# Healthcare-Robotics/assistive-gym

Hardware: NVIDIA H100
Metric: env-steps/sec FeedingJaco-v1 @batch4096 (higher is better)
Workload: dtype f32

## Files before the change

### assistive_gym_b200/capi.py

```python
import ctypes as C
import os

_HERE = os.path.dirname(os.path.abspath(__file__))
LIB_PATH = os.path.join(_HERE, 'csrc', 'libagphys.so')

P_I32 = C.POINTER(C.c_int32)
P_F64 = C.POINTER(C.c_double)
P_F32 = C.POINTER(C.c_float)


class AgConfig(C.Structure):
    _fields_ = [('dt', C.c_double), ('num_substeps', C.c_int), ('num_solver_iters', C.c_int),
                ('erp', C.c_double), ('contact_erp', C.c_double), ('linear_slop', C.c_double),
                ('residual_threshold', C.c_double), ('contact_threshold', C.c_double),
                ('linear_damping', C.c_double), ('angular_damping', C.c_double),
                ('max_coord_velocity', C.c_double), ('hull_margin', C.c_double),
                ('cone_friction', C.c_int), ('gyroscopic', C.c_int), ('max_contacts', C.c_int),
                ('warmstart_contact', C.c_double), ('warmstart_joint', C.c_double)]


def default_config(**kw):
    c = AgConfig(dt=0.02, num_substeps=1, num_solver_iters=50, erp=0.2, contact_erp=0.08, linear_slop=1e-5,
                 residual_threshold=1e-7, contact_threshold=0.02, linear_damping=0.04, angular_damping=0.04,
                 max_coord_velocity=100.0, hull_margin=0.001, cone_friction=1, gyroscopic=1, max_contacts=128,
# ... 228 lines not shown
    lib.ag_scratch_init.argtypes = [vp, C.POINTER(AgScratchParams), vp, vp, vp]
    lib.ag_scratch_step_dev.argtypes = [vp, vp, vp, vp, vp, vp]
    lib.ag_scratch_step_host.argtypes = [vp, vp, vp, vp, vp, vp]
    lib.ag_drinking_init.argtypes = [vp, C.POINTER(AgDrinkingParams), vp]
    lib.ag_drinking_step_dev.argtypes = [vp, vp, vp, vp, vp, vp]
    lib.ag_drinking_step_host.argtypes = [vp, vp, vp, vp, vp, vp]
    lib.ag_drinking_get_state.argtypes = [vp, vp, vp, vp]
    lib.ag_coop_init.argtypes = [vp, C.POINTER(AgCoopParams), vp, vp]
    lib.ag_coop_step_dev.argtypes = [vp, vp, vp, vp, vp, vp, vp]
    lib.ag_coop_step_host.argtypes = [vp, vp, vp, vp, vp, vp, vp]
    lib.ag_coop_classify.argtypes = [vp, ci, vp, vp]
    lib.ag_render.argtypes = [vp, C.POINTER(AgCamera), ci, vp, vp, vp]
    lib.ag_ik_solve.argtypes = [vp, ci, vp, ci, vp, vp, ci, ci, C.c_float, C.c_uint64, vp, vp, vp]
    lib.ag_state_size.restype = C.c_size_t
    lib.ag_state_size.argtypes = [vp]
    lib.ag_state_get.argtypes = [vp, vp]
    lib.ag_state_set.argtypes = [vp, vp]
    lib.ag_kernel_launches.restype = C.c_uint64
    lib.ag_kernel_launches.argtypes = [vp]
    lib.ag_overflow_count.argtypes = [vp]
    lib.ag_get_solver_stats.argtypes = [vp, vp, vp]
    lib.ag_get_pgs_cycles.argtypes = [vp, vp]
    lib.ag_get_pgs_trips.argtypes = [vp, vp, vp]
    lib.ag_get_pgs_occupancy.argtypes = [vp, vp, vp]
    lib.ag_profile_enable.argtypes = [vp, ci]
    lib.ag_profile_get.argtypes = [vp, ci, vp, ci, vp, vp]
    if path is None:
        _lib = lib
    return lib


EXPORTED_SYMBOLS = [
    'ag_last_error', 'ag_default_config', 'ag_create', 'ag_destroy', 'ag_num_envs', 'ag_stream',
    'ag_set_base_pose', 'ag_set_base_velocity', 'ag_set_joint_state', 'ag_set_link_friction',
    'ag_set_body_active', 'ag_forward_kinematics', 'ag_set_motor_host', 'ag_set_motor_targets_dev', 'ag_set_motor_targets_host',
    'ag_step', 'ag_get_joint_states', 'ag_get_link_states', 'ag_get_contacts', 'ag_contact_force_sum',
    'ag_closest_points', 'ag_feeding_init', 'ag_feeding_reset_episode', 'ag_feeding_set_tremor', 'ag_set_hard_limits', 'ag_feeding_step_dev', 'ag_ik_solve', 'ag_bathing_init', 'ag_bathing_step_dev', 'ag_bathing_step_host',
    'ag_feeding_step_host', 'ag_feeding_step_host_begin', 'ag_feeding_step_host_end', 'ag_state_size', 'ag_state_get', 'ag_state_set', 'ag_kernel_launches',
    'ag_cloth_init', 'ag_cloth_set_state', 'ag_cloth_get_state', 'ag_cloth_set_anchor', 'ag_cloth_anchor_follow', 'ag_cloth_set_gravity',
    'ag_cloth_get_contacts', 'ag_cloth_device_state', 'ag_scratch_init', 'ag_scratch_step_dev', 'ag_scratch_step_host', 'ag_render', 'ag_set_body_gravity', 'ag_get_link_aabb', 'ag_dressing_init', 'ag_dressing_reset_episode', 'ag_dressing_set_tremor', 'ag_set_motor_force_scale', 'ag_dressing_step_dev', 'ag_dressing_step_host',
    'ag_overflow_count', 'ag_get_solver_stats', 'ag_get_pgs_cycles', 'ag_get_pgs_trips', 'ag_get_pgs_occupancy', 'ag_profile_enable', 'ag_profile_get',
    'ag_coop_init', 'ag_coop_step_dev', 'ag_coop_step_host', 'ag_coop_classify', 'ag_bathing_set_target_frames',
    'ag_drinking_init', 'ag_drinking_step_dev', 'ag_drinking_step_host', 'ag_drinking_get_state',
]
```

### assistive_gym_b200/csrc/ag_device.cuh

```cuda
#pragma once
#include <string.h>
#include "ag_math.cuh"
#include "ag_types.h"

AG_HD float ld1(const float* p, int item, int N, int e) { return p[(size_t)item * N + e]; }
AG_HD void st1(float* p, int item, int N, int e, float v) { p[(size_t)item * N + e] = v; }
AG_HD f3 ld3(const float* p, int item, int N, int e) {
  size_t b = (size_t)item * 3 * N + e;
  return f3(p[b], p[b + N], p[b + 2 * (size_t)N]);
}
AG_HD void st3(float* p, int item, int N, int e, f3 v) {
  size_t b = (size_t)item * 3 * N + e;
  p[b] = v.x; p[b + N] = v.y; p[b + 2 * (size_t)N] = v.z;
}
AG_HD q4 ld4(const float* p, int item, int N, int e) {
  size_t b = (size_t)item * 4 * N + e;
  return q4(p[b], p[b + N], p[b + 2 * (size_t)N], p[b + 3 * (size_t)N]);
}
AG_HD void st4(float* p, int item, int N, int e, q4 v) {
  size_t b = (size_t)item * 4 * N + e;
  p[b] = v.x; p[b + N] = v.y; p[b + 2 * (size_t)N] = v.z; p[b + 3 * (size_t)N] = v.w;
}
AG_HD f3 tv3(const float* p, int i) { return f3(AG_LDG(p + 3 * i), AG_LDG(p + 3 * i + 1), AG_LDG(p + 3 * i + 2)); }
AG_HD q4 tv4(const float* p, int i) { return q4(AG_LDG(p + 4 * i), AG_LDG(p + 4 * i + 1), AG_LDG(p + 4 * i + 2), AG_LDG(p + 4 * i + 3)); }
// ... 98 lines not shown
AG_HD vq4 ldq4(const float* p) {
#if defined(__CUDA_ARCH__)
  float4 v = __ldg((const float4*)p); vq4 r; r.x = v.x; r.y = v.y; r.z = v.z; r.w = v.w; return r;
#else
  return *(const vq4*)p;
#endif
}
AG_HD int support4(const float* vq, int g0, int n, f3 d) {
  int bi = 0; float best = -3.0e38f;
  const int ng = (n + 3) >> 2;
  const float* p = vq + (size_t)g0 * 12;
  for (int g = 0; g < ng; g++, p += 12) {
    vq4 X = ldq4(p), Y = ldq4(p + 4), Z = ldq4(p + 8);
    float d0 = d.x * X.x + d.y * Y.x + d.z * Z.x, d1 = d.x * X.y + d.y * Y.y + d.z * Z.y;
    float d2 = d.x * X.z + d.y * Y.z + d.z * Z.z, d3v = d.x * X.w + d.y * Y.w + d.z * Z.w;
    if (d0 > best) { best = d0; bi = 4 * g; }
    if (d1 > best) { best = d1; bi = 4 * g + 1; }
    if (d2 > best) { best = d2; bi = 4 * g + 2; }
    if (d3v > best) { best = d3v; bi = 4 * g + 3; }
  }
  return bi < n ? bi : 0;
}

AG_HDN inline bool gjk_cores(const float* verts, const float* vq, int va0, int ga0, int nA, int vb0, int gb0, int nB, const m3& R, f3 t,
                             f3& pa, f3& pb, f3& nrm, float& dist) {
  d3 W[4]; f3 PA[4], PB[4];
  int IA[4], IB[4];
  double lam[4] = {1.0, 0.0, 0.0, 0.0};
  int n = 0;
  d3 v = to_d3(mul(R, tv3(verts, va0)) + t) - to_d3(tv3(verts, vb0));
  if (dot(v, v) < 1e-20) v = d3(1.0, 0.0, 0.0);
  bool overlap = false;
  double lower_bound = 0.0;
  for (int it = 0; it < 32; it++) {
    f3 vf = to_f3(v);
    f3 da = mulT(R, -vf);
    int ia = support4(vq, ga0, nA, da), ib = support4(vq, gb0, nB, vf);
    f3 sa = mul(R, tv3(verts, va0 + ia)) + t;
    f3 sb = tv3(verts, vb0 + ib);
    d3 w = to_d3(sa) - to_d3(sb);
    double vv = dot(v, v);
    double vw = dot(v, w);
    if (n > 0 && vw > 0.0) lower_bound = fmax(lower_bound, vw / sqrt(vv));
    if (n > 0 && vv - vw <= 1e-10 * vv) break;
    bool dup = false;
    for (int i = 0; i < n; i++) if (IA[i] == ia && IB[i] == ib) dup = true;
    if (dup) break;
    W[n] = w; PA[n] = sa; PB[n] = sb; IA[n] = ia; IB[n] = ib; n++;
    if (n == 1) { lam[0] = 1.0; }
    else if (n == 2) {
      double u, s; seg_origin(W[0], W[1], u, s);
      if (s <= 0.0) { n = 1; lam[0] = 1.0; }
      else if (u <= 0.0) { W[0] = W[1]; PA[0] = PA[1]; PB[0] = PB[1]; IA[0] = IA[1]; IB[0] = IB[1]; n = 1; lam[0] = 1.0; }
      else { lam[0] = u; lam[1] = s; }
    } else if (n == 3) {
      double l3[3]; tri_origin(W[0], W[1], W[2], l3[0], l3[1], l3[2]);
      int m = 0;
      for (int i = 0; i < 3; i++) if (l3[i] > 0.0) { W[m] = W[i]; PA[m] = PA[i]; PB[m] = PB[i]; IA[m] = IA[i]; IB[m] = IB[i]; lam[m] = l3[i]; m++; }
      n = m;
    } else {
      double bestd = 1e300; int bf = -1; double bl[3] = {0.0, 0.0, 0.0};
      double bestd_all = 1e300; int bf_all = 0; double bla[3] = {1.0, 0.0, 0.0};
      bool any_out = false;
      for (int f = 0; f < 4; f++) {
        int i0 = (f == 3) ? 1 : 0, i1 = (f == 0) ? 1 : ((f == 1) ? 2 : 3), i2 = (f == 0) ? 2 : ((f == 1) ? 3 : ((f == 2) ? 1 : 2)), i3 = (f == 0) ? 3 : ((f == 1) ? 1 : ((f == 2) ? 2 : 0));
        d3 a = W[i0], b = W[i1], c = W[i2], d = W[i3];
        d3 nn = cross(b - a, c - a);
        double sp = -dot(a, nn), sd = dot(d - a, nn);
        double nl = sqrt(dot(nn, nn));
        double tol_d = 1e-9 * nl * sqrt(dot(d - a, d - a)), tol_p = 1e-9 * nl * sqrt(dot(a, a));
        bool inside = (sp * sd > 0.0) && (fabs(sd) > tol_d) && (fabs(sp) > tol_p);
        double u, s, r; tri_origin(a, b, c, u, s, r);
        d3 pt = a * u + b * s + c * r;
        double dd = dot(pt, pt);
        if (dd < bestd_all) { bestd_all = dd; bf_all = f; bla[0] = u; bla[1] = s; bla[2] = r; }
        if (inside) continue;
        any_out = true;
        if (dd < bestd) { bestd = dd; bf = f; bl[0] = u; bl[1] = s; bl[2] = r; }
      }
      if (!any_out) {
        if (lower_bound <= 1e-7) { overlap = true; break; }
        bf = bf_all; bl[0] = bla[0]; bl[1] = bla[1]; bl[2] = bla[2];
      }
      int f = bf;
      int id[3];
      id[0] = (f == 3) ? 1 : 0; id[1] = (f == 0) ? 1 : ((f == 1) ? 2 : 3); id[2] = (f == 0) ? 2 : ((f == 1) ? 3 : ((f == 2) ? 1 : 2));
      d3 tw[3]; f3 ta[3], tb[3]; int tia[3], tib[3];
      for (int i = 0; i < 3; i++) { tw[i] = W[id[i]]; ta[i] = PA[id[i]]; tb[i] = PB[id[i]]; tia[i] = IA[id[i]]; tib[i] = IB[id[i]]; }
      int m = 0;
      for (int i = 0; i < 3; i++) if (bl[i] > 0.0) { W[m] = tw[i]; PA[m] = ta[i]; PB[m] = tb[i]; IA[m] = tia[i]; IB[m] = tib[i]; lam[m] = bl[i]; m++; }
      n = m;
    }
    d3 nv(0.0, 0.0, 0.0);
    for (int i = 0; i < n; i++) nv = nv + W[i] * lam[i];
    v = nv;
    if (dot(v, v) <= 1e-16) { overlap = true; break; }
  }
  if (overlap) return true;
  d3 qa(0.0, 0.0, 0.0), qb(0.0, 0.0, 0.0);
  for (int i = 0; i < n; i++) { qa = qa + to_d3(PA[i]) * lam[i]; qb = qb + to_d3(PB[i]) * lam[i]; }
  d3 d = qa - qb;
  double dn = sqrt(dot(d, d));
  pa = to_f3(qa); pb = to_f3(qb);
  dist = (float)dn;
  nrm = dn > 0.0 ? to_f3(d * (1.0 / dn)) : f3(0.f, 0.f, 1.f);
  return false;
}

AG_HDN inline void pen_faces(const SimDev& S, int va0, int nA, int pa0, int npA, int vb0, int nB, int pb0, int npB,
                             const m3& R, f3 t, f3& pa, f3& pb, f3& nrm, float& dist) {
  float best = -1e30f; bool found = false;
  for (int k = 0; k < npA; k++) {
    f3 nl; float dl; ld_plane(S.planes, pa0 + k, nl, dl);
    f3 n = mul(R, nl); float d = dl + dot(n, t);
    int jb = 0; float mn = dot(n, tv3(S.verts, vb0));
    for (int j = 1; j < nB; j++) { float x = dot(n, tv3(S.verts, vb0 + j)); if (x < mn) { mn = x; jb = j; } }
    float sep = mn - d;
    if (sep > best) { best = sep; found = true; nrm = -n; pb = tv3(S.verts, vb0 + jb); pa = pb - n * sep; }
  }
  for (int k = 0; k < npB; k++) {
    f3 n; float d; ld_plane(S.planes, pb0 + k, n, d);
    f3 nl = mulT(R, n);
    int ja = 0; float mn = dot(nl, tv3(S.verts, va0));
    for (int j = 1; j < nA; j++) { float x = dot(nl, tv3(S.verts, va0 + j)); if (x < mn) { mn = x; ja = j; } }
    float sep = mn + dot(n, t) - d;
    if (sep > best) { best = sep; found = true; nrm = n; pa = mul(R, tv3(S.verts, va0 + ja)) + t; pb = pa - n * sep; }
  }
  if (!found) { nrm = f3(0.f, 0.f, 1.f); pa = mul(R, tv3(S.verts, va0)) + t; pb = tv3(S.verts, vb0); best = 0.f; }
  dist = fminf(best, 0.f);
}

struct CandSet { NpOut c[4]; int n; };
struct CandSel {
  NpOut prim; NpOut pool[12]; int np;
};

AG_HDN inline void face_cands(const SimDev& S, int vv0, int nV, float rV, bool v_is_a, int p0, int np, float rP,
                              const m3& R, f3 t, f3 n_to_v, float d_primary, float tol, float max_dist, CandSel& cs) {
  int kf = -1; float best = 0.98f; f3 nf; float df = 0.f;
  for (int k = 0; k < np; k++) {
    f3 n; float d; ld_plane(S.planes, p0 + k, n, d);
    if (!v_is_a) { f3 nw = mul(R, n); d = d + dot(nw, t); n = nw; }
    float al = dot(n, n_to_v);
    if (al > best) { best = al; kf = k; nf = n; df = d; }
  }
  if (kf < 0) return;
  for (int i = 0; i < nV; i++) {
    f3 v = tv3(S.verts, vv0 + i);
    if (v_is_a) v = mul(R, v) + t;
    float h = dot(nf, v) - df;
    float d = h - rV - rP;
    if (d > d_primary + tol || d > max_dist) continue;
    f3 proj = v - nf * h;
    bool inside = true;
    for (int k = 0; k < np; k++) {
      if (k == kf) continue;
      f3 n; float dd; ld_plane(S.planes, p0 + k, n, dd);
      if (!v_is_a) { f3 nw = mul(R, n); dd = dd + dot(nw, t); n = nw; }
      if (dot(n, proj) - dd > 1e-6f) { inside = false; break; }
    }
    if (!inside) continue;
    if (cs.np >= 12) {
      int wi = 0; for (int q = 1; q < 12; q++) if (cs.pool[q].d > cs.pool[wi].d) wi = q;
      if (d >= cs.pool[wi].d) continue;
      cs.np = 12;
      NpOut& o = cs.pool[wi];
      f3 on_v = v - nf * rV, on_f = proj + nf * rP;
      if (v_is_a) { o.pa = on_v; o.pb = on_f; o.n = nf; } else { o.pa = on_f; o.pb = on_v; o.n = -nf; }
      o.d = d;
      continue;
    }
    NpOut& o = cs.pool[cs.np++];
    f3 on_v = v - nf * rV, on_f = proj + nf * rP;
    if (v_is_a) { o.pa = on_v; o.pb = on_f; o.n = nf; } else { o.pa = on_f; o.pb = on_v; o.n = -nf; }
    o.d = d;
  }
}

AG_HDN inline int select_cands(const CandSel& cs, NpOut* out) {
  if (cs.np == 0) { out[0] = cs.prim; return 1; }
  bool used[12];
  int first = 0;
  for (int i = 0; i < 12; i++) used[i] = i >= cs.np;
  for (int i = 1; i < cs.np; i++) if (cs.pool[i].d < cs.pool[first].d) first = i;
  int nc = 0; out[nc++] = cs.pool[first]; used[first] = true;
  while (nc < 4) {
    int bi = -1; float bd = 1e-8f;
    for (int i = 0; i < cs.np; i++) {
      if (used[i]) continue;
      float md = 1e30f;
      for (int k = 0; k < nc; k++) { f3 d = cs.pool[i].pa - out[k].pa; md = fminf(md, dot(d, d)); }
      if (md > bd) { bd = md; bi = i; }
    }
    if (bi < 0) break;
    used[bi] = true; out[nc++] = cs.pool[bi];
  }
  return nc;
}

AG_HDN inline int narrow_pair(const SimDev& S, int e, int ca, int cb, float max_dist, bool manifold, NpOut* out) {
  const int N = S.N;
  int ta = AG_LDG(S.col_type + ca), tb = AG_LDG(S.col_type + cb);
  float ra = AG_LDG(S.col_radius + ca), rb = AG_LDG(S.col_radius + cb);
  int ka = AG_LDG(S.col_link + ca), kb = AG_LDG(S.col_link + cb);
  int va0 = AG_LDG(S.col_v0 + ca), nA = AG_LDG(S.col_nv + ca), vb0 = AG_LDG(S.col_v0 + cb), nB = AG_LDG(S.col_nv + cb);
  int pa0 = AG_LDG(S.col_p0 + ca), npA = AG_LDG(S.col_np + ca), pb0 = AG_LDG(S.col_p0 + cb), npB = AG_LDG(S.col_np + cb);
  f3 posA = ld3(S.lpos, ka, N, e), posB = ld3(S.lpos, kb, N, e);
  q4 qA = ld4(S.lquat, ka, N, e), qB = ld4(S.lquat, kb, N, e);
  CandSel cs; cs.np = 0;
  int nout;
  if (ta == 3 || tb == 3) {
    if (ta == tb) return 0;
    bool flip = (ta == 3);
    q4 qP = flip ? qA : qB, qV = flip ? qB : qA;
    f3 pP = flip ? posA : posB, pV = flip ? posB : posA;
    m3 R = mul(transpose(qmat(qP)), qmat(qV));
    f3 t = qrot_inv(qP, pV - pP);
    int vv0 = flip ? vb0 : va0, nV = flip ? nB : nA; float rv = flip ? rb : ra;
    f3 pn; float pd; ld_plane(S.planes, flip ? pa0 : pb0, pn, pd);
    int j = 0; float mn = 1e30f;
    for (int i = 0; i < nV; i++) { float x = dot(pn, mul(R, tv3(S.verts, vv0 + i)) + t); if (x < mn) { mn = x; j = i; } }
    float d = mn - pd - rv;
    if (d > max_dist) return 0;
    f3 vj = mul(R, tv3(S.verts, vv0 + j)) + t;
    cs.prim.pa = vj - pn * rv; cs.prim.pb = vj - pn * (mn - pd); cs.prim.n = pn; cs.prim.d = d;
    if (manifold && nV > 1) face_cands(S, vv0, nV, rv, true, flip ? pa0 : pb0, 1, 0.f, R, t, pn, d, max_dist * 0.5f, max_dist, cs);
    nout = select_cands(cs, out);
    m3 RP = qmat(qP);
    for (int i = 0; i < nout; i++) {
      f3 a = mul(RP, out[i].pa) + pP, b = mul(RP, out[i].pb) + pP, n = mul(RP, out[i].n);
      if (!flip) { out[i].pa = a; out[i].pb = b; out[i].n = n; }
      else { out[i].pa = b; out[i].pb = a; out[i].n = -n; }
    }
    return nout;
  }
  m3 RB = qmat(qB);
  m3 R = mul(transpose(RB), qmat(qA));
  f3 t = mulT(RB, posA - posB);
  f3 pa, pb, nrm; float dist = 0.f;
  bool ov = gjk_cores(S.verts, S.vertq, va0, AG_LDG(S.col_g0 + ca), nA, vb0, AG_LDG(S.col_g0 + cb), nB, R, t, pa, pb, nrm, dist);
  if (ov) pen_faces(S, va0, nA, pa0, npA, vb0, nB, pb0, npB, R, t, pa, pb, nrm, dist);
  float d = dist - ra - rb;
  if (d > max_dist) return 0;
  cs.prim.n = nrm; cs.prim.pa = pa - nrm * ra; cs.prim.pb = pb + nrm * rb; cs.prim.d = d;
  if (manifold) {
    if (npB > 0 && nA > 1) face_cands(S, va0, nA, ra, true, pb0, npB, rb, R, t, nrm, d, max_dist * 0.5f, max_dist, cs);
    if (npA > 0 && nB > 1) face_cands(S, vb0, nB, rb, false, pa0, npA, ra, R, t, -nrm, d, max_dist * 0.5f, max_dist, cs);
  }
  nout = select_cands(cs, out);
  for (int i = 0; i < nout; i++) {
    out[i].pa = mul(RB, out[i].pa) + posB; out[i].pb = mul(RB, out[i].pb) + posB; out[i].n = mul(RB, out[i].n);
  }
  return nout;
}

AG_HD int ag_atomic_inc(int* p) {
#if defined(__CUDA_ARCH__)
  return atomicAdd(p, 1);
#else
  int v = *p; *p = v + 1; return v;
#endif
}
AG_HD int ag_atomic_add(int* p, int k) {
#if defined(__CUDA_ARCH__)
  return atomicAdd(p, k);
#else
  int v = *p; *p = v + k; return v;
#endif
}

AG_HDN inline void pairs_body(int tid, const SimDev& S, const KP& kp) {
  const int N = S.N;
  int Npad = kp.i0;
// ... 12 lines not shown
    float tha = AG_LDG(S.col_thresh + ca);
    if (!aabb_ov(amin, amax, lbmin, lbmax, fac * fminf(tha, tlb))) continue;
    for (int cb = cb0; cb < cb0 + ncb; cb++) {
      float thr = fac * fminf(tha, AG_LDG(S.col_thresh + cb));
      if (!aabb_ov(amin, amax, ld3(S.cmin, cb, N, e), ld3(S.cmax, cb, N, e), thr)) continue;
      int slot = ag_atomic_inc(S.cand_count + e);
      int cost = AG_LDG(S.col_nv + ca) + AG_LDG(S.col_nv + cb); if (cost > 255) cost = 255;
      if (slot < S.maxcand) S.cand[(size_t)slot * N + e] = ((unsigned)(255 - cost) << 24) | ((unsigned)ca * (unsigned)S.nc + (unsigned)cb);
    }
  }
}

AG_HDN inline void csort_body(int tid, const SimDev& S, const KP&) {
  const int N = S.N;
  int e = tid % N, cs = tid / N;
  int n = S.cand_count[e]; if (n > S.maxcand) n = S.maxcand;
  if (cs >= n) return;
  unsigned w = S.cand[(size_t)cs * N + e];
  int rank = 0;
  for (int j = 0; j < n; j++) rank += (S.cand[(size_t)j * N + e] < w) ? 1 : 0;
  S.cand_s[(size_t)rank * N + e] = w;
}

AG_HDN inline void narrow_body(int tid, const SimDev& S, const KP&) {
  const int N = S.N;
  int e = tid % N, cs = tid / N;
  int ncand = S.cand_count[e]; if (ncand > S.maxcand) ncand = S.maxcand;
  if (cs >= ncand) return;
  unsigned pk = S.cand_s[(size_t)cs * N + e] & 0xffffffu;
  int ca = (int)(pk / (unsigned)S.nc), cb = (int)(pk % (unsigned)S.nc);
  float thr = S.contact_thr * fminf(AG_LDG(S.col_thresh + ca), AG_LDG(S.col_thresh + cb));
  NpOut out[4];
  int n = narrow_pair(S, e, ca, cb, thr, true, out);
  for (int i = 0; i < n; i++) {
    int slot = ag_atomic_inc(S.c_count + e);
    if (slot >= S.maxraw) continue;
    S.c_key[(size_t)slot * N + e] = pk * 4u + (unsigned)i;
    float* c = S.c_data + (size_t)slot * AG_CFR * N + e;
    c[(size_t)CF_PAX * N] = out[i].pa.x; c[(size_t)CF_PAY * N] = out[i].pa.y; c[(size_t)CF_PAZ * N] = out[i].pa.z;
    c[(size_t)CF_PBX * N] = out[i].pb.x; c[(size_t)CF_PBY * N] = out[i].pb.y; c[(size_t)CF_PBZ * N] = out[i].pb.z;
    c[(size_t)CF_NX * N] = out[i].n.x; c[(size_t)CF_NY * N] = out[i].n.y; c[(size_t)CF_NZ * N] = out[i].n.z;
    c[(size_t)CF_DIST * N] = out[i].d;
  }
}

AG_HD void contact_refs(const SimDev& S, int e, unsigned key, int& refA, int& refB);
AG_HDN inline void sort_body(int tid, const SimDev& S, const KP&) {
  const int N = S.N;
  int e = tid % N, slot = tid / N;
  int cnt = S.c_count[e];
  int n = cnt < S.maxraw ? cnt : S.maxraw;
  if (slot == 0 && ((cnt > S.maxc) || (S.cand_count[e] > S.maxcand))) S.overflow[e] = 1;
  if (slot >= n) return;
  unsigned key = S.c_key[(size_t)slot * N + e];
  int rank = 0;
  for (int j = 0; j < n; j++) rank += (S.c_key[(size_t)j * N + e] < key) ? 1 : 0;
  if (rank >= S.maxc) return;
  S.s_key[(size_t)rank * N + e] = key;
  { int ra, rb2; contact_refs(S, e, key, ra, rb2); S.s_ref[(size_t)rank * 4 * N + e] = ra; S.s_ref[((size_t)rank * 4 + 1) * N + e] = rb2; }
  for (int f = 0; f <= CF_DIST; f++) cf_st(S.s_data, rank, f, N, e, S.c_data[((size_t)slot * AG_CFR + f) * N + e]);
}

struct AI { s3 A; m3 B; s3 D; };
struct SVf { f3 a, l; };

AG_HD SVf ai_mul(const AI& I, SVf v) {
  SVf r;
// ... 226 lines not shown
```

### assistive_gym_b200/csrc/agphys.cu

```cuda
#include <stdio.h>
#include <stdlib.h>
#include <string.h>
#include <string>
#include <vector>
#include <algorithm>
#include "../../include/agphys.h"
#include "ag_device.cuh"
#include "ag_solver.cuh"
#include "ag_feeding.cuh"
#include "ag_bathing.cuh"
#include "ag_ik.cuh"
#include "ag_cloth.cuh"
#include "ag_dressing.cuh"
#include "ag_render.cuh"
#include "ag_scratch.cuh"
#include "ag_coop.cuh"
#include "ag_drinking.cuh"

#ifndef AG_CPU_EMU
#include <cuda_runtime.h>
#define AG_GLOBAL __global__
#else
#define AG_GLOBAL
typedef void* cudaStream_t;
// ... 8 lines not shown
    int tid = blockIdx.x * blockDim.x + threadIdx.x;                            \
    if (tid < p.n) body(tid, S, p);                                             \
  }
#else
#define AG_KERNEL(name, body) \
  static void name(SimDev S, KP p) { for (int tid = 0; tid < p.n; tid++) body(tid, S, p); }
#endif

#ifndef AG_CPU_EMU
#define AG_KERNEL_B(name, body, minblocks)                                      \
  __global__ void __launch_bounds__(128, minblocks) name(SimDev S, KP p) {      \
    int tid = blockIdx.x * blockDim.x + threadIdx.x;                            \
    if (tid < p.n) body(tid, S, p);                                             \
  }
#else
#define AG_KERNEL_B(name, body, minblocks) AG_KERNEL(name, body)
#endif
AG_KERNEL(k_fk, fk_body)
AG_KERNEL(k_aabb, aabb_body)
AG_KERNEL(k_linkaabb, linkaabb_body)
AG_KERNEL(k_pairs, pairs_body)
AG_KERNEL(k_csort, csort_body)
AG_KERNEL_B(k_narrow, narrow_body, 3)
AG_KERNEL(k_sort, sort_body)
AG_KERNEL(k_dyn, dyn_body)
AG_KERNEL(k_rows, rows_body)
AG_KERNEL(k_crows, crows_body)
#ifndef AG_CPU_EMU
__global__ void __launch_bounds__(32) k_pgs(SimDev S, KP p) {
  extern __shared__ __align__(128) float pgs_smem[];
  pgs_warp(S, pgs_smem, p.i0, blockIdx.x * RS_CTA_ENVS);
}
__global__ void __launch_bounds__(1024) k_order(SimDev S, KP) {
  __shared__ int hist[64];
  if (threadIdx.x < 64) hist[threadIdx.x] = 0;
  __syncthreads();
  for (int e = threadIdx.x; e < S.N; e += blockDim.x) atomicAdd(&hist[pgs_work_bucket(S, e)], 1);
  __syncthreads();
  if (threadIdx.x == 0) { int acc = 0; for (int b = 0; b < 64; b++) { int c = hist[b]; hist[b] = acc; acc += c; } }
  __syncthreads();
  for (int e = threadIdx.x; e < S.N; e += blockDim.x) S.pgs_order[atomicAdd(&hist[pgs_work_bucket(S, e)], 1)] = e;
}
#else
static void k_pgs(SimDev S, KP p) {
  std::vector<float> buf((size_t)rs_env_floats(S) + 8);
  float* base = (float*)(((uintptr_t)buf.data() + 15) & ~(uintptr_t)15);
// ... 883 lines not shown
    const float* o = in + sz * e;
    for (int b = 0; b < s->nb; b++) {
      for (int a = 0; a < 3; a++) { bp[((size_t)b * 3 + a) * N + e] = o[a]; bl[((size_t)b * 3 + a) * N + e] = o[7 + a]; ba[((size_t)b * 3 + a) * N + e] = o[10 + a]; }
      for (int a = 0; a < 4; a++) bq[((size_t)b * 4 + a) * N + e] = o[3 + a];
      o += 13;
    }
    for (int k = 0; k < s->nl; k++) { q[(size_t)k * N + e] = o[0]; qd[(size_t)k * N + e] = o[1]; o += 2; }
  }
  if (h2d(s, s->S.base_pos, bp.data(), bp.size() * 4) || h2d(s, s->S.base_quat, bq.data(), bq.size() * 4) ||
      h2d(s, s->S.base_lin, bl.data(), bl.size() * 4) || h2d(s, s->S.base_ang, ba.data(), ba.size() * 4) ||
      h2d(s, s->S.jq, q.data(), q.size() * 4) || h2d(s, s->S.jqd, qd.data(), qd.size() * 4)) return -1;
  run_fk_all(s);
  return 0;
}

int ag_get_pgs_cycles(AgSim* s, int32_t* cycles) {
  DevGuard guard__(s->device); return d2h(s, cycles, s->S.pgs_cycles, sizeof(int) * s->S.N); }
int ag_get_pgs_trips(AgSim* s, int32_t* trips, int32_t* stream_floats) {
  DevGuard guard__(s->device);
  if (trips && d2h(s, trips, s->S.pgs_trips, sizeof(int) * s->S.N)) return -1;
  if (stream_floats && d2h(s, stream_floats, s->S.rs_nfloats, sizeof(int) * s->S.N)) return -1;
  return 0;
}
int ag_get_pgs_occupancy(AgSim* s, int32_t* ctas_per_sm, int32_t* smem_bytes) {
  DevGuard guard__(s->device);
  const size_t smem = (size_t)rs_cta_floats(s->S) * sizeof(float);
  int ctas = 0;
#ifndef AG_CPU_EMU
  if (cudaOccupancyMaxActiveBlocksPerMultiprocessor(&ctas, k_pgs, 32, smem) != cudaSuccess) return fail("cudaOccupancyMaxActiveBlocksPerMultiprocessor(k_pgs) failed");
#endif
  if (ctas_per_sm) *ctas_per_sm = ctas;
  if (smem_bytes) *smem_bytes = (int32_t)smem;
  return 0;
}

int ag_get_solver_stats(AgSim* s, int32_t* contacts, int32_t* iters) {
  DevGuard guard__(s->device);
  if (contacts && d2h(s, contacts, s->S.c_count, sizeof(int) * s->S.N)) return -1;
  if (iters && d2h(s, iters, s->S.iters_used, sizeof(int) * s->S.N)) return -1;
  return 0;
}

int ag_overflow_count(AgSim* s) {
  DevGuard guard__(s->device);
  std::vector<int> o(s->S.N);
  if (d2h(s, o.data(), s->S.overflow, sizeof(int) * s->S.N)) return -1;
// ... 843 lines not shown
```

### assistive_gym_b200/sim.py

```python
import ctypes as C

import numpy as np

from . import capi


def _p(a):
    return None if a is None else a.ctypes.data_as(C.c_void_p)


def _f32(a, shape=None):
    if a is None:
        return None
    a = np.asarray(a, dtype=np.float32)
    if shape is not None:
        a = np.broadcast_to(a, shape)
    return np.ascontiguousarray(a)


def _i32(a):
    return None if a is None else np.ascontiguousarray(a, dtype=np.int32)


_OBS_W = {'feeding': (25, 23), 'scratch': (30, 34), 'bathing': (24, 28), 'dressing': (24, 28), 'drinking': (25, 0)}
# ... 130 lines not shown

    def kernel_launches(self):
        return int(self.lib.ag_kernel_launches(self.h))

    def overflow_count(self):
        return int(self.lib.ag_overflow_count(self.h))

    def solver_stats(self):
        c, it = np.zeros(self.n, dtype=np.int32), np.zeros(self.n, dtype=np.int32)
        self._ck(self.lib.ag_get_solver_stats(self.h, _p(c), _p(it)))
        return c, it

    def pgs_cycles(self):
        c = np.zeros(self.n, dtype=np.int32)
        self._ck(self.lib.ag_get_pgs_cycles(self.h, _p(c)))
        return c

    def pgs_trips(self):
        t = np.zeros(self.n, dtype=np.int32)
        f = np.zeros(self.n, dtype=np.int32)
        self._ck(self.lib.ag_get_pgs_trips(self.h, _p(t), _p(f)))
        return t, f

    def pgs_occupancy(self):
        c, b = C.c_int32(0), C.c_int32(0)
        self._ck(self.lib.ag_get_pgs_occupancy(self.h, C.byref(c), C.byref(b)))
        return c.value, b.value

    def profile_enable(self, on=True):
        self._ck(self.lib.ag_profile_enable(self.h, int(bool(on))))

    def profile_get(self):
        mx, stride = 32, 48
        names = C.create_string_buffer(mx * stride)
        ms = np.zeros(mx, dtype=np.float32)
        cnt = np.zeros(mx, dtype=np.int32)
        n = self.lib.ag_profile_get(self.h, mx, names, stride, _p(ms), _p(cnt))
        out = {}
        for i in range(max(n, 0)):
            nm = names.raw[i * stride:(i + 1) * stride].split(b'\0')[0].decode()
            out[nm] = (float(ms[i]), int(cnt[i]))
        return out

    def stream_ptr(self):
        return int(self.lib.ag_stream(self.h) or 0)

# ... 233 lines not shown
```

### include/agphys.h

```cpp
#ifndef AGPHYS_H
#define AGPHYS_H
#include <stddef.h>
#include <stdint.h>

#ifdef __cplusplus
extern "C" {
#endif

enum { AG_JOINT_FIXED = 0, AG_JOINT_REVOLUTE = 1, AG_JOINT_PRISMATIC = 2,
       AG_JOINT_FREE_BASE = 3, AG_JOINT_FIXED_BASE = 4 };
enum { AG_COL_SPHERE = 0, AG_COL_CAPSULE = 1, AG_COL_HULL = 2, AG_COL_HALFSPACE = 3 };
enum { AG_MOTOR_OFF = 0, AG_MOTOR_POSITION = 1, AG_MOTOR_VELOCITY = 2 };

typedef struct AgConfig {
  double dt;
  int    num_substeps;
  int    num_solver_iters;
  double erp;
  double contact_erp;
  double linear_slop;
  double residual_threshold;
  double contact_threshold;
  double linear_damping;
  double angular_damping;
// ... 251 lines not shown
  float eye[3], target[3], up[3];
  float fov_deg, aspect, near_, far_;
  int32_t width, height;
  float light_dir[3];
  float ambient, diffuse;
} AgCamera;
int ag_render(AgSim* sim, const AgCamera* cam, int n, const int32_t* env_ids, uint8_t* rgba, float* depth);

int ag_ik_solve(AgSim* sim, int n_joints, const int32_t* joint_links, int ee_link, const float* target_pos,
                const float* target_quat, int max_restarts, int iters, float threshold, uint64_t seed,
                const int32_t* env_mask, float* q_out, float* err_out);

size_t ag_state_size(const AgSim* sim);
int    ag_state_get(AgSim* sim, float* out);
int    ag_state_set(AgSim* sim, const float* in);

uint64_t ag_kernel_launches(const AgSim* sim);
int      ag_profile_enable(AgSim* sim, int on);
int      ag_profile_get(AgSim* sim, int max_names, char* names, int name_stride, float* total_ms, int32_t* counts);
int      ag_overflow_count(AgSim* sim);
int      ag_get_solver_stats(AgSim* sim, int32_t* contacts, int32_t* iters);
int      ag_get_pgs_cycles(AgSim* sim, int32_t* cycles);
int      ag_get_pgs_trips(AgSim* sim, int32_t* trips, int32_t* stream_floats);
int      ag_get_pgs_occupancy(AgSim* sim, int32_t* ctas_per_sm, int32_t* smem_bytes);

#ifdef __cplusplus
}
#endif
#endif
```

Before: 361,300.

## Keep GJK simplex and manifold candidates in registers; add narrow-phase probe

```diff
diff --git a/assistive_gym_b200/capi.py b/assistive_gym_b200/capi.py
--- a/assistive_gym_b200/capi.py
+++ b/assistive_gym_b200/capi.py
@@ -274,6 +274,8 @@
     lib.ag_get_solver_stats.argtypes = [vp, vp, vp]
     lib.ag_get_pgs_cycles.argtypes = [vp, vp]
     lib.ag_get_pgs_trips.argtypes = [vp, vp, vp]
+    lib.ag_get_narrow_candidates.argtypes = [vp, vp]
+    lib.ag_narrow_probe.argtypes = [vp, ci, vp, vp, vp]
     lib.ag_get_pgs_occupancy.argtypes = [vp, vp, vp]
     lib.ag_profile_enable.argtypes = [vp, ci]
     lib.ag_profile_get.argtypes = [vp, ci, vp, ci, vp, vp]
@@ -291,7 +293,7 @@
     'ag_feeding_step_host', 'ag_feeding_step_host_begin', 'ag_feeding_step_host_end', 'ag_state_size', 'ag_state_get', 'ag_state_set', 'ag_kernel_launches',
     'ag_cloth_init', 'ag_cloth_set_state', 'ag_cloth_get_state', 'ag_cloth_set_anchor', 'ag_cloth_anchor_follow', 'ag_cloth_set_gravity',
     'ag_cloth_get_contacts', 'ag_cloth_device_state', 'ag_scratch_init', 'ag_scratch_step_dev', 'ag_scratch_step_host', 'ag_render', 'ag_set_body_gravity', 'ag_get_link_aabb', 'ag_dressing_init', 'ag_dressing_reset_episode', 'ag_dressing_set_tremor', 'ag_set_motor_force_scale', 'ag_dressing_step_dev', 'ag_dressing_step_host',
-    'ag_overflow_count', 'ag_get_solver_stats', 'ag_get_pgs_cycles', 'ag_get_pgs_trips', 'ag_get_pgs_occupancy', 'ag_profile_enable', 'ag_profile_get',
+    'ag_overflow_count', 'ag_get_solver_stats', 'ag_get_pgs_cycles', 'ag_get_pgs_trips', 'ag_get_narrow_candidates', 'ag_narrow_probe', 'ag_get_pgs_occupancy', 'ag_profile_enable', 'ag_profile_get',
     'ag_coop_init', 'ag_coop_step_dev', 'ag_coop_step_host', 'ag_coop_classify', 'ag_bathing_set_target_frames',
     'ag_drinking_init', 'ag_drinking_step_dev', 'ag_drinking_step_host', 'ag_drinking_get_state',
 ]
diff --git a/assistive_gym_b200/csrc/ag_device.cuh b/assistive_gym_b200/csrc/ag_device.cuh
--- a/assistive_gym_b200/csrc/ag_device.cuh
+++ b/assistive_gym_b200/csrc/ag_device.cuh
@@ -144,10 +144,12 @@
   return bi < n ? bi : 0;
 }
 
+struct GjkVtx { d3 w; int ia, ib; };
+AG_HD f3 gjk_sup_a(const float* verts, int va0, int i, const m3& R, f3 t) { return mul(R, tv3(verts, va0 + i)) + t; }
+
 AG_HDN inline bool gjk_cores(const float* verts, const float* vq, int va0, int ga0, int nA, int vb0, int gb0, int nB, const m3& R, f3 t,
                              f3& pa, f3& pb, f3& nrm, float& dist) {
-  d3 W[4]; f3 PA[4], PB[4];
-  int IA[4], IB[4];
+  GjkVtx V[4];
   double lam[4] = {1.0, 0.0, 0.0, 0.0};
   int n = 0;
   d3 v = to_d3(mul(R, tv3(verts, va0)) + t) - to_d3(tv3(verts, vb0));
@@ -158,7 +160,7 @@
     f3 vf = to_f3(v);
     f3 da = mulT(R, -vf);
     int ia = support4(vq, ga0, nA, da), ib = support4(vq, gb0, nB, vf);
-    f3 sa = mul(R, tv3(verts, va0 + ia)) + t;
+    f3 sa = gjk_sup_a(verts, va0, ia, R, t);
     f3 sb = tv3(verts, vb0 + ib);
     d3 w = to_d3(sa) - to_d3(sb);
     double vv = dot(v, v);
@@ -166,27 +168,37 @@
     if (n > 0 && vw > 0.0) lower_bound = fmax(lower_bound, vw / sqrt(vv));
     if (n > 0 && vv - vw <= 1e-10 * vv) break;
     bool dup = false;
-    for (int i = 0; i < n; i++) if (IA[i] == ia && IB[i] == ib) dup = true;
+#pragma unroll
+    for (int i = 0; i < 4; i++) if (i < n && V[i].ia == ia && V[i].ib == ib) dup = true;
     if (dup) break;
-    W[n] = w; PA[n] = sa; PB[n] = sb; IA[n] = ia; IB[n] = ib; n++;
+    GjkVtx nv_ = {w, ia, ib};
+#pragma unroll
+    for (int q = 0; q < 4; q++) if (q == n) V[q] = nv_;
+    n++;
     if (n == 1) { lam[0] = 1.0; }
     else if (n == 2) {
-      double u, s; seg_origin(W[0], W[1], u, s);
+      double u, s; seg_origin(V[0].w, V[1].w, u, s);
       if (s <= 0.0) { n = 1; lam[0] = 1.0; }
-      else if (u <= 0.0) { W[0] = W[1]; PA[0] = PA[1]; PB[0] = PB[1]; IA[0] = IA[1]; IB[0] = IB[1]; n = 1; lam[0] = 1.0; }
+      else if (u <= 0.0) { V[0] = V[1]; n = 1; lam[0] = 1.0; }
       else { lam[0] = u; lam[1] = s; }
     } else if (n == 3) {
-      double l3[3]; tri_origin(W[0], W[1], W[2], l3[0], l3[1], l3[2]);
+      double l3[3]; tri_origin(V[0].w, V[1].w, V[2].w, l3[0], l3[1], l3[2]);
       int m = 0;
-      for (int i = 0; i < 3; i++) if (l3[i] > 0.0) { W[m] = W[i]; PA[m] = PA[i]; PB[m] = PB[i]; IA[m] = IA[i]; IB[m] = IB[i]; lam[m] = l3[i]; m++; }
+#pragma unroll
+      for (int i = 0; i < 3; i++) if (l3[i] > 0.0) {
+#pragma unroll
+        for (int q = 0; q <= i; q++) if (q == m) { V[q] = V[i]; lam[q] = l3[i]; }
+        m++;
+      }
       n = m;
     } else {
       double bestd = 1e300; int bf = -1; double bl[3] = {0.0, 0.0, 0.0};
       double bestd_all = 1e300; int bf_all = 0; double bla[3] = {1.0, 0.0, 0.0};
       bool any_out = false;
+#pragma unroll
       for (int f = 0; f < 4; f++) {
         int i0 = (f == 3) ? 1 : 0, i1 = (f == 0) ? 1 : ((f == 1) ? 2 : 3), i2 = (f == 0) ? 2 : ((f == 1) ? 3 : ((f == 2) ? 1 : 2)), i3 = (f == 0) ? 3 : ((f == 1) ? 1 : ((f == 2) ? 2 : 0));
-        d3 a = W[i0], b = W[i1], c = W[i2], d = W[i3];
+        d3 a = V[i0].w, b = V[i1].w, c = V[i2].w, d = V[i3].w;
         d3 nn = cross(b - a, c - a);
         double sp = -dot(a, nn), sd = dot(d - a, nn);
         double nl = sqrt(dot(nn, nn));
@@ -204,23 +216,32 @@
         if (lower_bound <= 1e-7) { overlap = true; break; }
         bf = bf_all; bl[0] = bla[0]; bl[1] = bla[1]; bl[2] = bla[2];
       }
-      int f = bf;
-      int id[3];
-      id[0] = (f == 3) ? 1 : 0; id[1] = (f == 0) ? 1 : ((f == 1) ? 2 : 3); id[2] = (f == 0) ? 2 : ((f == 1) ? 3 : ((f == 2) ? 1 : 2));
-      d3 tw[3]; f3 ta[3], tb[3]; int tia[3], tib[3];
-      for (int i = 0; i < 3; i++) { tw[i] = W[id[i]]; ta[i] = PA[id[i]]; tb[i] = PB[id[i]]; tia[i] = IA[id[i]]; tib[i] = IB[id[i]]; }
+      GjkVtx tv[3];
+#pragma unroll
+      for (int f = 0; f < 4; f++) if (f == bf) {
+        tv[0] = V[(f == 3) ? 1 : 0]; tv[1] = V[(f == 0) ? 1 : ((f == 1) ? 2 : 3)]; tv[2] = V[(f == 0) ? 2 : ((f == 1) ? 3 : ((f == 2) ? 1 : 2))];
+      }
       int m = 0;
-      for (int i = 0; i < 3; i++) if (bl[i] > 0.0) { W[m] = tw[i]; PA[m] = ta[i]; PB[m] = tb[i]; IA[m] = tia[i]; IB[m] = tib[i]; lam[m] = bl[i]; m++; }
+#pragma unroll
+      for (int i = 0; i < 3; i++) if (bl[i] > 0.0) {
+#pragma unroll
+        for (int q = 0; q <= i; q++) if (q == m) { V[q] = tv[i]; lam[q] = bl[i]; }
+        m++;
+      }
       n = m;
     }
     d3 nv(0.0, 0.0, 0.0);
-    for (int i = 0; i < n; i++) nv = nv + W[i] * lam[i];
+#pragma unroll
+    for (int i = 0; i < 4; i++) if (i < n) nv = nv + V[i].w * lam[i];
     v = nv;
     if (dot(v, v) <= 1e-16) { overlap = true; break; }
   }
   if (overlap) return true;
   d3 qa(0.0, 0.0, 0.0), qb(0.0, 0.0, 0.0);
-  for (int i = 0; i < n; i++) { qa = qa + to_d3(PA[i]) * lam[i]; qb = qb + to_d3(PB[i]) * lam[i]; }
+#pragma unroll
+  for (int i = 0; i < 4; i++) if (i < n) {
+    qa = qa + to_d3(gjk_sup_a(verts, va0, V[i].ia, R, t)) * lam[i]; qb = qb + to_d3(tv3(verts, vb0 + V[i].ib)) * lam[i];
+  }
   d3 d = qa - qb;
   double dn = sqrt(dot(d, d));
   pa = to_f3(qa); pb = to_f3(qb);
@@ -253,12 +274,42 @@
 }
 
 struct CandSet { NpOut c[4]; int n; };
+struct CandFace { f3 nf; float df, rV, rP; int vv0; bool v_is_a; };
 struct CandSel {
-  NpOut prim; NpOut pool[12]; int np;
+  NpOut prim; CandFace face[2]; int key[12]; float d[12]; int np;
 };
 
-AG_HDN inline void face_cands(const SimDev& S, int vv0, int nV, float rV, bool v_is_a, int p0, int np, float rP,
-                              const m3& R, f3 t, f3 n_to_v, float d_primary, float tol, float max_dist, CandSel& cs) {
+#if defined(__CUDA_ARCH__)
+AG_HD f3 sub_fused(f3 a, f3 b, float s) { return f3(__fmaf_rn(-b.x, s, a.x), __fmaf_rn(-b.y, s, a.y), __fmaf_rn(-b.z, s, a.z)); }
+AG_HD f3 sub_mul(f3 a, f3 b, float s) { return f3(__fsub_rn(a.x, __fmul_rn(b.x, s)), __fsub_rn(a.y, __fmul_rn(b.y, s)), __fsub_rn(a.z, __fmul_rn(b.z, s))); }
+AG_HD f3 add_mul(f3 a, f3 b, float s) { return f3(__fadd_rn(a.x, __fmul_rn(b.x, s)), __fadd_rn(a.y, __fmul_rn(b.y, s)), __fadd_rn(a.z, __fmul_rn(b.z, s))); }
+#else
+AG_HD f3 sub_fused(f3 a, f3 b, float s) { return a - b * s; }
+AG_HD f3 sub_mul(f3 a, f3 b, float s) { return a - b * s; }
+AG_HD f3 add_mul(f3 a, f3 b, float s) { return a + b * s; }
+#endif
+
+AG_HD f3 face_vertex(const SimDev& S, const CandFace& F, int i, const m3& R, f3 t, float& h) {
+  f3 v = tv3(S.verts, F.vv0 + i);
+  if (F.v_is_a) v = mul(R, v) + t;
+  h = dot(F.nf, v) - F.df;
+  return v;
+}
+
+AG_HD NpOut cand_point(const SimDev& S, const CandSel& cs, int key, float d, const m3& R, f3 t) {
+  CandFace F = cs.face[0];
+  if (key & 1) F = cs.face[1];
+  float h; f3 v = face_vertex(S, F, key >> 1, R, t, h);
+  f3 proj = sub_fused(v, F.nf, h);
+  f3 on_v = sub_mul(v, F.nf, F.rV), on_f = add_mul(proj, F.nf, F.rP);
+  NpOut o;
+  if (F.v_is_a) { o.pa = on_v; o.pb = on_f; o.n = F.nf; } else { o.pa = on_f; o.pb = on_v; o.n = -F.nf; }
+  o.d = d;
+  return o;
+}
+
+AG_HD void face_cands(const SimDev& S, int call, int vv0, int nV, float rV, bool v_is_a, int p0, int np, float rP,
+                      const m3& R, f3 t, f3 n_to_v, float d_primary, float tol, float max_dist, CandSel& cs) {
   int kf = -1; float best = 0.98f; f3 nf; float df = 0.f;
   for (int k = 0; k < np; k++) {
     f3 n; float d; ld_plane(S.planes, p0 + k, n, d);
@@ -267,13 +318,13 @@
     if (al > best) { best = al; kf = k; nf = n; df = d; }
   }
   if (kf < 0) return;
+  CandFace F; F.nf = nf; F.df = df; F.rV = rV; F.rP = rP; F.vv0 = vv0; F.v_is_a = v_is_a;
+  cs.face[call] = F;
   for (int i = 0; i < nV; i++) {
-    f3 v = tv3(S.verts, vv0 + i);
-    if (v_is_a) v = mul(R, v) + t;
-    float h = dot(nf, v) - df;
+    float h; f3 v = face_vertex(S, F, i, R, t, h);
     float d = h - rV - rP;
     if (d > d_primary + tol || d > max_dist) continue;
-    f3 proj = v - nf * h;
+    f3 proj = sub_fused(v, nf, h);
     bool inside = true;
     for (int k = 0; k < np; k++) {
       if (k == kf) continue;
@@ -282,45 +333,63 @@
       if (dot(n, proj) - dd > 1e-6f) { inside = false; break; }
     }
     if (!inside) continue;
+    int slot = cs.np;
     if (cs.np >= 12) {
-      int wi = 0; for (int q = 1; q < 12; q++) if (cs.pool[q].d > cs.pool[wi].d) wi = q;
-      if (d >= cs.pool[wi].d) continue;
-      cs.np = 12;
-      NpOut& o = cs.pool[wi];
-      f3 on_v = v - nf * rV, on_f = proj + nf * rP;
-      if (v_is_a) { o.pa = on_v; o.pb = on_f; o.n = nf; } else { o.pa = on_f; o.pb = on_v; o.n = -nf; }
-      o.d = d;
-      continue;
-    }
-    NpOut& o = cs.pool[cs.np++];
-    f3 on_v = v - nf * rV, on_f = proj + nf * rP;
-    if (v_is_a) { o.pa = on_v; o.pb = on_f; o.n = nf; } else { o.pa = on_f; o.pb = on_v; o.n = -nf; }
-    o.d = d;
-  }
-}
-
-AG_HDN inline int select_cands(const CandSel& cs, NpOut* out) {
+      int wi = 0; float wd = cs.d[0];
+#pragma unroll
+      for (int q = 1; q < 12; q++) if (cs.d[q] > wd) { wd = cs.d[q]; wi = q; }
+      if (d >= wd) continue;
+      slot = wi;
+    } else {
+      cs.np++;
+    }
+#pragma unroll
+    for (int q = 0; q < 12; q++) if (q == slot) { cs.key[q] = 2 * i + call; cs.d[q] = d; }
+  }
+}
+
+AG_HD int select_cands(const SimDev& S, const CandSel& cs, const m3& R, f3 t, NpOut* out) {
   if (cs.np == 0) { out[0] = cs.prim; return 1; }
-  bool used[12];
-  int first = 0;
-  for (int i = 0; i < 12; i++) used[i] = i >= cs.np;
-  for (int i = 1; i < cs.np; i++) if (cs.pool[i].d < cs.pool[first].d) first = i;
-  int nc = 0; out[nc++] = cs.pool[first]; used[first] = true;
-  while (nc < 4) {
-    int bi = -1; float bd = 1e-8f;
-    for (int i = 0; i < cs.np; i++) {
-      if (used[i]) continue;
-      float md = 1e30f;
-      for (int k = 0; k < nc; k++) { f3 d = cs.pool[i].pa - out[k].pa; md = fminf(md, dot(d, d)); }
-      if (md > bd) { bd = md; bi = i; }
+  f3 pa[12];
+#pragma unroll
+  for (int i = 0; i < 12; i++) if (i < cs.np) pa[i] = cand_point(S, cs, cs.key[i], cs.d[i], R, t).pa;
+  int first = 0; int pk[4]; float pd[4]; f3 last = pa[0];
+  pk[0] = cs.key[0]; pd[0] = cs.d[0];
+#pragma unroll
+  for (int i = 1; i < 12; i++) if (i < cs.np && cs.d[i] < pd[0]) { first = i; pk[0] = cs.key[i]; pd[0] = cs.d[i]; last = pa[i]; }
+  unsigned used = ((0xfffu << cs.np) | (1u << first)) & 0xfffu;
+  float md[12];
+#pragma unroll
+  for (int i = 0; i < 12; i++) md[i] = 1e30f;
+  int nc = 1;
+#pragma unroll
+  for (int r = 1; r < 4; r++) {
+    int bi = -1; float bd = 1e-8f; f3 bpa;
+#pragma unroll
+    for (int i = 0; i < 12; i++) {
+      if ((used >> i) & 1u) continue;
+      f3 d = pa[i] - last; md[i] = fminf(md[i], dot(d, d));
+      if (md[i] > bd) { bd = md[i]; bi = i; bpa = pa[i]; pk[r] = cs.key[i]; pd[r] = cs.d[i]; }
     }
     if (bi < 0) break;
-    used[bi] = true; out[nc++] = cs.pool[bi];
-  }
+    used |= 1u << bi; last = bpa; nc = r + 1;
+  }
+#pragma unroll
+  for (int r = 0; r < 4; r++) if (r < nc) out[r] = cand_point(S, cs, pk[r], pd[r], R, t);
   return nc;
 }
 
-AG_HDN inline int narrow_pair(const SimDev& S, int e, int ca, int cb, float max_dist, bool manifold, NpOut* out) {
+enum { NPC_GJK, NPC_PEN, NPC_MANIFOLD, NPC_TOTAL, NPC_N };
+AG_HD long long ag_clock() {
+#if defined(__CUDA_ARCH__)
+  return clock64();
+#else
+  return 0;
+#endif
+}
+
+template <bool TIMED = false>
+AG_HDN inline int narrow_pair(const SimDev& S, int e, int ca, int cb, float max_dist, bool manifold, NpOut* out, long long* cyc = nullptr) {
   const int N = S.N;
   int ta = AG_LDG(S.col_type + ca), tb = AG_LDG(S.col_type + cb);
   float ra = AG_LDG(S.col_radius + ca), rb = AG_LDG(S.col_radius + cb);
@@ -329,7 +398,7 @@
   int pa0 = AG_LDG(S.col_p0 + ca), npA = AG_LDG(S.col_np + ca), pb0 = AG_LDG(S.col_p0 + cb), npB = AG_LDG(S.col_np + cb);
   f3 posA = ld3(S.lpos, ka, N, e), posB = ld3(S.lpos, kb, N, e);
   q4 qA = ld4(S.lquat, ka, N, e), qB = ld4(S.lquat, kb, N, e);
-  CandSel cs; cs.np = 0;
+  CandSel cs; cs.np = 0; cs.face[0] = cs.face[1] = CandFace();
   int nout;
   if (ta == 3 || tb == 3) {
     if (ta == tb) return 0;
@@ -346,10 +415,13 @@
     if (d > max_dist) return 0;
     f3 vj = mul(R, tv3(S.verts, vv0 + j)) + t;
     cs.prim.pa = vj - pn * rv; cs.prim.pb = vj - pn * (mn - pd); cs.prim.n = pn; cs.prim.d = d;
-    if (manifold && nV > 1) face_cands(S, vv0, nV, rv, true, flip ? pa0 : pb0, 1, 0.f, R, t, pn, d, max_dist * 0.5f, max_dist, cs);
-    nout = select_cands(cs, out);
+    long long t0 = TIMED ? ag_clock() : 0;
+    if (manifold && nV > 1) face_cands(S, 0, vv0, nV, rv, true, flip ? pa0 : pb0, 1, 0.f, R, t, pn, d, max_dist * 0.5f, max_dist, cs);
+    nout = select_cands(S, cs, R, t, out);
+    if (TIMED) cyc[NPC_MANIFOLD] += ag_clock() - t0;
     m3 RP = qmat(qP);
-    for (int i = 0; i < nout; i++) {
+#pragma unroll
+    for (int i = 0; i < 4; i++) if (i < nout) {
       f3 a = mul(RP, out[i].pa) + pP, b = mul(RP, out[i].pb) + pP, n = mul(RP, out[i].n);
       if (!flip) { out[i].pa = a; out[i].pb = b; out[i].n = n; }
       else { out[i].pa = b; out[i].pb = a; out[i].n = -n; }
@@ -360,17 +432,22 @@
   m3 R = mul(transpose(RB), qmat(qA));
   f3 t = mulT(RB, posA - posB);
   f3 pa, pb, nrm; float dist = 0.f;
+  long long t0 = TIMED ? ag_clock() : 0;
   bool ov = gjk_cores(S.verts, S.vertq, va0, AG_LDG(S.col_g0 + ca), nA, vb0, AG_LDG(S.col_g0 + cb), nB, R, t, pa, pb, nrm, dist);
+  if (TIMED) { long long t1 = ag_clock(); cyc[NPC_GJK] += t1 - t0; t0 = t1; }
   if (ov) pen_faces(S, va0, nA, pa0, npA, vb0, nB, pb0, npB, R, t, pa, pb, nrm, dist);
+  if (TIMED) { long long t1 = ag_clock(); cyc[NPC_PEN] += t1 - t0; t0 = t1; }
   float d = dist - ra - rb;
   if (d > max_dist) return 0;
   cs.prim.n = nrm; cs.prim.pa = pa - nrm * ra; cs.prim.pb = pb + nrm * rb; cs.prim.d = d;
   if (manifold) {
-    if (npB > 0 && nA > 1) face_cands(S, va0, nA, ra, true, pb0, npB, rb, R, t, nrm, d, max_dist * 0.5f, max_dist, cs);
-    if (npA > 0 && nB > 1) face_cands(S, vb0, nB, rb, false, pa0, npA, ra, R, t, -nrm, d, max_dist * 0.5f, max_dist, cs);
-  }
-  nout = select_cands(cs, out);
-  for (int i = 0; i < nout; i++) {
+    if (npB > 0 && nA > 1) face_cands(S, 0, va0, nA, ra, true, pb0, npB, rb, R, t, nrm, d, max_dist * 0.5f, max_dist, cs);
+    if (npA > 0 && nB > 1) face_cands(S, 1, vb0, nB, rb, false, pa0, npA, ra, R, t, -nrm, d, max_dist * 0.5f, max_dist, cs);
+  }
+  nout = select_cands(S, cs, R, t, out);
+  if (TIMED) cyc[NPC_MANIFOLD] += ag_clock() - t0;
+#pragma unroll
+  for (int i = 0; i < 4; i++) if (i < nout) {
     out[i].pa = mul(RB, out[i].pa) + posB; out[i].pb = mul(RB, out[i].pb) + posB; out[i].n = mul(RB, out[i].n);
   }
   return nout;
@@ -429,7 +506,16 @@
   S.cand_s[(size_t)rank * N + e] = w;
 }
 
-AG_HDN inline void narrow_body(int tid, const SimDev& S, const KP&) {
+AG_HD void ag_atomic_add64(long long* p, long long k) {
+#if defined(__CUDA_ARCH__)
+  atomicAdd((unsigned long long*)p, (unsigned long long)k);
+#else
+  *p += k;
+#endif
+}
+
+template <bool TIMED>
+AG_HDN inline void narrow_body_t(int tid, const SimDev& S, const KP& p) {
   const int N = S.N;
   int e = tid % N, cs = tid / N;
   int ncand = S.cand_count[e]; if (ncand > S.maxcand) ncand = S.maxcand;
@@ -438,8 +524,11 @@
   int ca = (int)(pk / (unsigned)S.nc), cb = (int)(pk % (unsigned)S.nc);
   float thr = S.contact_thr * fminf(AG_LDG(S.col_thresh + ca), AG_LDG(S.col_thresh + cb));
   NpOut out[4];
-  int n = narrow_pair(S, e, ca, cb, thr, true, out);
-  for (int i = 0; i < n; i++) {
+  long long cyc[NPC_N] = {0, 0, 0, 0};
+  long long t_begin = TIMED ? ag_clock() : 0;
+  int n = narrow_pair<TIMED>(S, e, ca, cb, thr, true, out, cyc);
+#pragma unroll
+  for (int i = 0; i < 4; i++) if (i < n) {
     int slot = ag_atomic_inc(S.c_count + e);
     if (slot >= S.maxraw) continue;
     S.c_key[(size_t)slot * N + e] = pk * 4u + (unsigned)i;
@@ -449,7 +538,13 @@
     c[(size_t)CF_NX * N] = out[i].n.x; c[(size_t)CF_NY * N] = out[i].n.y; c[(size_t)CF_NZ * N] = out[i].n.z;
     c[(size_t)CF_DIST * N] = out[i].d;
   }
-}
+  if (TIMED) {
+    cyc[NPC_TOTAL] = ag_clock() - t_begin;
+    for (int k = 0; k < NPC_N; k++) ag_atomic_add64((long long*)p.p0 + (size_t)k * N + e, cyc[k]);
+  }
+}
+AG_HDN inline void narrow_body(int tid, const SimDev& S, const KP& p) { narrow_body_t<false>(tid, S, p); }
+AG_HDN inline void narrow_timed_body(int tid, const SimDev& S, const KP& p) { narrow_body_t<true>(tid, S, p); }
 
 AG_HD void contact_refs(const SimDev& S, int e, unsigned key, int& refA, int& refB);
 AG_HDN inline void sort_body(int tid, const SimDev& S, const KP&) {
diff --git a/assistive_gym_b200/csrc/agphys.cu b/assistive_gym_b200/csrc/agphys.cu
--- a/assistive_gym_b200/csrc/agphys.cu
+++ b/assistive_gym_b200/csrc/agphys.cu
@@ -54,6 +54,7 @@
 AG_KERNEL(k_pairs, pairs_body)
 AG_KERNEL(k_csort, csort_body)
 AG_KERNEL_B(k_narrow, narrow_body, 3)
+AG_KERNEL_B(k_narrow_timed, narrow_timed_body, 3)
 AG_KERNEL(k_sort, sort_body)
 AG_KERNEL(k_dyn, dyn_body)
 AG_KERNEL(k_rows, rows_body)
@@ -983,6 +984,55 @@
   if (stream_floats && d2h(s, stream_floats, s->S.rs_nfloats, sizeof(int) * s->S.N)) return -1;
   return 0;
 }
+int ag_get_narrow_candidates(AgSim* s, int32_t* candidates) {
+  DevGuard guard__(s->device); return d2h(s, candidates, s->S.cand_count, sizeof(int) * s->S.N); }
+
+int ag_narrow_probe(AgSim* s, int reps, float* ms, int32_t* live_slots, int64_t* cycles) {
+  DevGuard guard__(s->device);
+  SimDev& S = s->S;
+  const int N = S.N;
+  if (reps < 1) return fail("ag_narrow_probe: reps must be >= 1");
+  std::vector<int> cand(N), c_count(N);
+  if (d2h(s, cand.data(), S.cand_count, sizeof(int) * N) || d2h(s, c_count.data(), S.c_count, sizeof(int) * N)) return -1;
+  int live = 0;
+  for (int c : cand) live = std::max(live, std::min(c, S.maxcand));
+  if (live_slots) *live_slots = live;
+  long long* cyc = (long long*)dev_alloc(s, sizeof(long long) * NPC_N * N);
+  if (!cyc) return fail("ag_narrow_probe: out of device memory");
+  KP z = kp0(); KP zt = kp0(); zt.p0 = cyc;
+  const size_t grid[3] = {(size_t)S.maxcand * N, (size_t)live * N, (size_t)S.maxcand * N};
+  for (int k = 0; k < 3; k++) {
+    float t = 0.f;
+#ifndef AG_CPU_EMU
+    cudaEvent_t e0, e1;
+    CK(cudaEventCreate(&e0)); CK(cudaEventCreate(&e1));
+#endif
+    for (int r = 0; r < (k == 2 ? 1 : reps); r++) {
+      if (dev_zero(s, S.c_count, sizeof(int) * N)) return -1;
+#ifndef AG_CPU_EMU
+      CK(cudaEventRecord(e0, s->stream));
+#endif
+      if (k == 2) LAUNCH(s, k_narrow_timed, grid[k], zt); else LAUNCH(s, k_narrow, grid[k], z);
+#ifndef AG_CPU_EMU
+      CK(cudaEventRecord(e1, s->stream)); CK(cudaEventSynchronize(e1));
+      float dt = 0.f; CK(cudaEventElapsedTime(&dt, e0, e1)); t += dt;
+#endif
+    }
+#ifndef AG_CPU_EMU
+    cudaEventDestroy(e0); cudaEventDestroy(e1);
+#endif
+    if (ms) ms[k] = t / (k == 2 ? 1 : reps);
+  }
+  int rc = cycles ? d2h(s, cycles, cyc, sizeof(long long) * NPC_N * N) : 0;
+  if (!rc) rc = h2d(s, S.c_count, c_count.data(), sizeof(int) * N);
+#ifndef AG_CPU_EMU
+  cudaStreamSynchronize(s->stream); cudaFree(cyc);
+#else
+  free(cyc);
+#endif
+  s->allocs.erase(std::find(s->allocs.begin(), s->allocs.end(), (void*)cyc));
+  return rc;
+}
 int ag_get_pgs_occupancy(AgSim* s, int32_t* ctas_per_sm, int32_t* smem_bytes) {
   DevGuard guard__(s->device);
   const size_t smem = (size_t)rs_cta_floats(s->S) * sizeof(float);
diff --git a/assistive_gym_b200/sim.py b/assistive_gym_b200/sim.py
--- a/assistive_gym_b200/sim.py
+++ b/assistive_gym_b200/sim.py
@@ -176,6 +176,18 @@
         self._ck(self.lib.ag_get_pgs_trips(self.h, _p(t), _p(f)))
         return t, f
 
+    def narrow_candidates(self):
+        c = np.zeros(self.n, dtype=np.int32)
+        self._ck(self.lib.ag_get_narrow_candidates(self.h, _p(c)))
+        return c
+
+    def narrow_probe(self, reps=20):
+        ms = np.zeros(3, dtype=np.float32)
+        live = C.c_int32(0)
+        cyc = np.zeros((4, self.n), dtype=np.int64)
+        self._ck(self.lib.ag_narrow_probe(self.h, int(reps), _p(ms), C.byref(live), _p(cyc)))
+        return float(ms[0]), float(ms[1]), float(ms[2]), live.value, cyc
+
     def pgs_occupancy(self):
         c, b = C.c_int32(0), C.c_int32(0)
         self._ck(self.lib.ag_get_pgs_occupancy(self.h, C.byref(c), C.byref(b)))
diff --git a/include/agphys.h b/include/agphys.h
--- a/include/agphys.h
+++ b/include/agphys.h
@@ -297,6 +297,8 @@
 int      ag_get_solver_stats(AgSim* sim, int32_t* contacts, int32_t* iters);
 int      ag_get_pgs_cycles(AgSim* sim, int32_t* cycles);
 int      ag_get_pgs_trips(AgSim* sim, int32_t* trips, int32_t* stream_floats);
+int      ag_get_narrow_candidates(AgSim* sim, int32_t* candidates);
+int      ag_narrow_probe(AgSim* sim, int reps, float* ms, int32_t* live_slots, int64_t* cycles);
 int      ag_get_pgs_occupancy(AgSim* sim, int32_t* ctas_per_sm, int32_t* smem_bytes);
 
 #ifdef __cplusplus
```

New measurement: 373,700 (median of 6 runs). +3.4%, better.
